# dmMaze/comic-text-detector

Measured on AMD Instinct MI355X. Metric: pages/sec at 1024x1024 bs=32 (end-to-end detector, device-resident pages), higher is better.
Workload: dtype f16

## Files before the change

### comic-text-detector_amd/_lib.py

```python
from __future__ import annotations

import ctypes as C
import os
import subprocess

_HERE = os.path.dirname(os.path.abspath(__file__))
LIB_PATH = os.path.join(_HERE, "libctd_hip.so")
SELFTEST_PATH = os.path.join(_HERE, "ctd_selftest")

ABI_VERSION = 6
OK = 0
PREC_F32, PREC_F16, PREC_F32S = 0, 1, 2
ACT = {"none": 0, "silu": 1, "leaky": 2, "relu": 3, "sigmoid": 4}
IN_NCHW_F32, IN_NHWC_U8 = 0, 1
(OP_INPUT, OP_CONV, OP_CONVT, OP_MAXPOOL, OP_AVGPOOL2, OP_DETECT, OP_EXPORT, OP_STEM, OP_SEG_FINAL,
 OP_DB_UP) = range(1, 11)
OUT_MASK, OUT_LINES = 0, 1


class CtdTensor(C.Structure):
    _fields_ = [("channels", C.c_int32), ("log2_down", C.c_int32), ("dtype", C.c_int32)]


class CtdOp(C.Structure):
    _fields_ = [
# ... 47 lines not shown
    "ctd_nms_workspace_bytes": (C.c_size_t, [_i32, _i32]),
    "ctd_nms": (_i32, [_vp, _i32, _i32, _i32, _f, _f, _i32, _i32, _f, _vp, _vp, _vp, C.c_size_t, _vp]),
    "ctd_db_step": (_i32, [_vp, _i32, _i32, _i32, _f, _vp, _vp, _f, _vp]),
    "ctd_ccl_workspace_bytes": (C.c_size_t, [_i32, _i32, _i32]),
    "ctd_ccl": (_i32, [_vp, _i32, _i32, _i32, _i32, _i32, _vp, _vp, _vp, _i32, _vp, C.c_size_t, _vp]),
    "ctd_ccl_dual": (_i32, [_vp, _i32, _i32, _i32, _i32, _vp, _vp, _vp, _vp, _vp, _vp, _vp, _i32, _vp, C.c_size_t, _vp]),
    "ctd_resize_linear_u8": (_i32, [_vp, _i32, _i32, _i32, _vp, _i32, _i32, _i32, _i32, _vp]),
    "ctd_db_boxes": (_i32, [_vp, _vp, _vp, _i32, _vp, _vp, _i32, _i32, _i32, _i32, C.c_double, _vp, _vp, C.POINTER(_i32)]),
    "ctd_tail_create": (_i32, [C.POINTER(_vp), _i32]),
    "ctd_tail_destroy": (None, [_vp]),
    "ctd_tail_stream": (_vp, [_vp]),
    "ctd_tail_run": (_i32, [_vp, _i32, _i32, _i32, _vp, _i32, _i32, _vp, _vp, _i64, _vp, C.POINTER(CtdTailPage),
                            C.POINTER(CtdTailParams), _vp, _vp, _vp]),
    "ctd_tail_timings": (_i32, [_vp, C.POINTER(C.c_double)]),
    "ctd_tail_refine_paths": (_i32, [_vp, C.POINTER(_i32)]),
    "ctd_tail_db_boxes": (_i32, [_vp, _i32, _i32, _i32, _vp, _i64, _vp, _i32, C.c_double]),
    "ctd_tail_refine": (_i32, [_vp, _i32, C.POINTER(CtdTailPage), _vp, _vp, _vp, _i32, _i32, _vp, _vp]),
    "ctd_tail_page_counts": (_i32, [_vp, _i32, C.POINTER(_i32), C.POINTER(_i32), C.POINTER(_i32), C.POINTER(_i32),
                                    C.POINTER(_i32)]),
    "ctd_tail_page_fetch": (_i32, [_vp, _i32, _vp, _vp, _vp, _vp, _vp, _vp, _vp, _vp]),
    "ctd_tail_batch_counts": (_i32, [_vp, _vp]),
    "ctd_tail_batch_fetch": (_i32, [_vp, _vp, _vp, _vp]),
    "ctd_tail_pack_records": (_i32, [_vp, _i32, _i32, _vp]),
    "ctd_tail_set_threads": (_i32, [_vp, _i32]),
    "ctd_db_boxes_compact": (_i32, [_i32, _i32, _i32, _vp, _vp, _vp, _vp, _vp, _i32, _vp, _vp, _vp, _vp, _vp, _vp, _vp, _vp,
                                    _vp, _i32, C.c_double, _vp, _vp, C.POINTER(_i32)]),
    "ctd_topk_colors": (_i32, [_vp, _vp]),
    "ctd_otsu_from_hist": (_i32, [_vp]),
    "ctd_inrange_bounds": (None, [C.c_double, C.c_double, C.POINTER(_i32), C.POINTER(_i32)]),
    "ctd_group_output": (_i32, [_vp, _vp, _i32, _vp, _i32, _i32, _i32, _vp, _i32, _vp, _i32, _vp, _i32, _vp, _i32,
# ... 70 lines not shown
```

### comic-text-detector_amd/csrc/engine.hip

```cpp
#include <algorithm>
#include <cmath>
#include <cstdio>
#include <cstdlib>
#include <cstring>
#include <string>
#include <vector>

#include "kernels.h"

namespace {

thread_local std::string g_err;

int fail(int code, const std::string& msg) {
  g_err = msg;
  return code;
}

#define HIP_TRY(expr)                                                                              \
  do {                                                                                             \
    hipError_t _e = (expr);                                                                        \
    if (_e != hipSuccess)                                                                          \
      return fail(CTD_ERR_HIP, std::string(#expr) + ": " + hipGetErrorString(_e));                 \
  } while (0)
// ... 1024 lines not shown

int ctd_fail_msg(int code, const std::string& msg) { return fail(code, msg); }
extern int g_tail_priority;
extern int g_tail_cus, g_tail_cu_first;
extern long long g_tail_dma_min;
#ifdef CTD_MEASURE_KNOBS
extern int g_tail_skip_pages;
extern int g_tail_ablate;
#endif
extern int g_tail_chain;
extern int g_tail_fused_rounds;
extern long long g_tail_fused_max_pix;
extern int g_tail_lds, g_tail_lds_rcap, g_tw_lds_runs_x10, g_tw_lds_threads;
extern long long g_tail_lds_cls0, g_tail_lds_cls1;
extern long long g_tail_lds_max_bytes;

extern "C" {

const char* ctd_last_error(void) { return g_err.c_str(); }
int32_t ctd_abi_version(void) { return CTD_ABI_VERSION; }

int ctd_device_info(int32_t device, char* name, int32_t* cu_count, int64_t* hbm_bytes) {
  hipDeviceProp_t p;
  HIP_TRY(hipGetDeviceProperties(&p, device));
  if (name) { std::strncpy(name, p.name, 255); name[255] = 0; }
  if (cu_count) *cu_count = p.multiProcessorCount;
  if (hbm_bytes) *hbm_bytes = (int64_t)p.totalGlobalMem;
  int arch = 0;
  const char* g = std::strstr(p.gcnArchName, "gfx");
  if (g) arch = std::atoi(g + 3);
// ... 137 lines not shown
  }
  return CTD_OK;
}

int64_t ctd_engine_workspace_bytes(const ctd_engine* e) { return e ? (int64_t)e->arena_bytes : 0; }
int32_t ctd_engine_arena_generation(const ctd_engine* e) { return e ? e->arena_gen : -1; }

int ctd_tuning_set(const char* key, int64_t value) {
  const std::string k = key ? key : "";
  if (k == "fuse") g_fuse = (int)value;
  else if (k == "tail_max_blocks") g_tail_max_blocks = (int)std::max<int64_t>(1, value);
  else if (k == "tail_chain") g_tail_chain = (int)value;
  else if (k == "tail_fused_rounds") g_tail_fused_rounds = (int)value;
  else if (k == "tail_fused_max_pix") g_tail_fused_max_pix = value;
  else if (k == "tail_lds") g_tail_lds = (int)value;
  else if (k == "tail_lds_rcap") g_tail_lds_rcap = (int)value;
  else if (k == "tail_lds_max_bytes") g_tail_lds_max_bytes = value;
  else if (k == "tail_lds_runs_x10") g_tw_lds_runs_x10 = (int)std::max<int64_t>(1, value);
  else if (k == "tail_lds_threads") g_tw_lds_threads = (int)value;
  else if (k == "tail_lds_cls0") g_tail_lds_cls0 = value;
  else if (k == "tail_lds_cls1") g_tail_lds_cls1 = value;
  else if (k == "tail_dma_min") g_tail_dma_min = value;
#ifdef CTD_MEASURE_KNOBS
  else if (k == "tail_skip_page_download") g_tail_skip_pages = value != 0;
  else if (k == "tail_ablate") g_tail_ablate = (int)value;
#endif
  else if (k == "tail_priority") g_tail_priority = (int)value;
  else if (k == "tail_cus") g_tail_cus = (int)value;
  else if (k == "tail_cu_first") g_tail_cu_first = (int)value;
  else if (k == "no_reuse") g_no_reuse = (int)value;
// ... 89 lines not shown
```

### comic-text-detector_amd/csrc/tail.h

```cpp
#pragma once
#include "ctd_common.h"

extern int g_tail_max_blocks;

struct DbcTables {
  int B, H, W, cap, rcap;
  const float* prob;
  long long prob_stride;
  const int* lab;
  const int* n_f;
  const int* n_b;
  const int* st_f;
  const int* st_b;
  const int* first_f;
  const int* first_b;
  int* par_f;
  int* par_b;
  int* off_f;
  int* off_b;
  int* hdr;
  int* row_lo;
  int* row_hi;
  double* sum_f;
  double* sum_b;
  double* ring_sum;
  int* ring_cnt;
};
void launch_dbc(const DbcTables& t, hipStream_t st);

struct TWin {
  const uint8_t* img;
  const uint8_t* mask;
  uint8_t* out;
  int img_w, mask_w, out_w;
  int x1, y1, w, h;
  int mx, my;
  int band0, nband;
};
struct TRule {
  int kind;
  int lo, hi;
};
struct TBand {
// ... 49 lines not shown
```

### comic-text-detector_amd/csrc/tail.hip

```cpp
#include <algorithm>
#include <atomic>
#include <chrono>
#include <mutex>
#include <cmath>
#include <cstring>
#include <string>
#include <thread>
#include <vector>

#include "host_refine.h"
#include "kernels.h"
#include "tail.h"

int ctd_fail_msg(int code, const std::string& msg);
int g_tail_priority = 1;
int g_tail_cus = 0, g_tail_cu_first = 0;

#define T_TRY(expr)                                                                                  \
  do {                                                                                               \
    hipError_t e_ = (expr);                                                                          \
    if (e_ != hipSuccess) return ctd_fail_msg(CTD_ERR_HIP, std::string(#expr) + ": " + hipGetErrorString(e_)); \
  } while (0)

namespace {
// ... 56 lines not shown
  std::vector<double> dist;
  std::vector<int16_t> db_boxes;
  std::vector<float> db_scores;
  std::vector<int32_t> yolo;
  std::vector<int32_t> yolo_cls;
  std::vector<float> yolo_conf;
};

struct WinReq {
  int page, x1, y1, x2, y2;
};

constexpr int kMaxDet = 300;
constexpr int kCompCap = 1 << 16;
constexpr int kRowCap = 1 << 18;

inline size_t align_up(size_t v, size_t a) { return (v + a - 1) / a * a; }

template <class F>
void parallel_for(int n, int max_threads, F f) {
  const int nt = std::min(max_threads, n);
  if (nt <= 1) {
    for (int i = 0; i < n; ++i) f(i);
    return;
  }
  std::atomic<int> next{0};
  auto work = [&]() {
    for (int i; (i = next.fetch_add(1)) < n;) f(i);
  };
  std::vector<std::thread> th;
  th.reserve(nt - 1);
  for (int k = 1; k < nt; ++k) th.emplace_back(work);
  work();
  for (auto& x : th) x.join();
}

}
int g_tail_chain = 1;
int g_tail_fused_rounds = 1;
long long g_tail_fused_max_pix = 100000;
int g_tail_lds = 1, g_tail_lds_rcap = 0;
long long g_tail_lds_max_bytes = 150 << 10;
long long g_tail_lds_cls0 = 40 << 10, g_tail_lds_cls1 = 80 << 10;
namespace {
struct ChainState {
  std::mutex mu;
  hipEvent_t last = nullptr;
  hipEvent_t ring[16] = {};
  unsigned next = 0;
};
constexpr int kChainDevices = 64;
inline ChainState* chain_state(int device) {
  static ChainState states[kChainDevices];
  return device >= 0 && device < kChainDevices ? &states[device] : nullptr;
}
struct GpuChain {
  hipStream_t st;
  ChainState* cs;
// ... 77 lines not shown
    return nullptr;
  }
  if (a.type == hipMemoryTypeHost && a.devicePointer) return a.devicePointer;
  return nullptr;
}

inline double now_ms() {
  return std::chrono::duration<double, std::milli>(std::chrono::steady_clock::now().time_since_epoch()).count();
}

}

struct ctd_tail {
  int device = 0;
  hipStream_t st = nullptr;
  DevBuf d_dets, d_nms_ws, d_lab_f, d_ccl_ws, d_ccl_small, d_dbc_i, d_dbc_d, d_rows, d_pmask, d_refined;
  DevBuf d_wins, d_rules, d_bands, d_hist, d_sums, d_canvas, d_clab, d_cstats, d_cnt, d_merged, d_mlab, d_mstats, d_cnt2, d_small, d_crop;
  DevBuf d_wins_c, d_bands_c, d_lds;
  PinBuf h_dets, h_hdr, h_tab, h_pmask, h_refined, h_hist, h_sums, h_wins, h_rules, h_bands, h_small, h_lab;
  PinBuf h_wins_c, h_bands_c, h_lds;
  int B = 0;
  std::vector<ctd_tail_page> pages;
  std::vector<size_t> poff;
  std::vector<uint8_t*> hmask;
  size_t ptotal = 0;
  std::vector<PageOut> out;
  double ms_stage[10] = {0, 0, 0, 0, 0, 0, 0, 0, 0, 0};
  double ms_db_wait = 0;
  double ms_sub[5] = {0, 0, 0, 0, 0};
  int host_threads = 8;
  int n_lds = 0, n_canvas = 0, n_ovf = 0;
  long long lds_per_block = 64 << 10;
  double ms_lds_wait = 0;
};

namespace {

struct Packed {
  std::vector<int> x, y;
  int W = 0, H = 0;
};
void shelf_pack(const std::vector<int>& w, const std::vector<int>& h, int min_width, Packed& out) {
  const int n = (int)w.size();
  out.x.assign(n, 0);
  out.y.assign(n, 0);
  int cw = min_width;
  for (int i = 0; i < n; ++i) cw = std::max(cw, w[i]);
  std::vector<int> order(n);
// ... 390 lines not shown
  const double w0 = now_ms();
  T_TRY(hipStreamSynchronize(st));
  t->ms_sub[3] = now_ms() - w0;
  return CTD_OK;
}

struct DbStage {
  int B = 0, Hn = 0, Wn = 0;
  const float* prob = nullptr;
  long long prob_stride = 0;
  int *lab = nullptr, *n_f = nullptr, *n_b = nullptr, *st_f = nullptr, *st_b = nullptr;
  int *first_f = nullptr, *first_b = nullptr, *par_f = nullptr, *par_b = nullptr, *off_f = nullptr, *off_b = nullptr;
  int *hdr = nullptr, *ring_cnt = nullptr, *row_lo = nullptr, *row_hi = nullptr;
  double *sum_f = nullptr, *sum_b = nullptr, *ring_sum = nullptr;
  int* hhdr = nullptr;
};

int db_enqueue(ctd_tail* t, DbStage& d, int B, int Hn, int Wn, const float* prob_dev, long long prob_stride,
               const uint8_t* bitmap_dev, Batch& pre, Batch& post) {
  hipStream_t st = t->st;
  const size_t hw = (size_t)Hn * Wn;
  const int cap = kCompCap, rcap = kRowCap;
  d.B = B, d.Hn = Hn, d.Wn = Wn, d.prob = prob_dev, d.prob_stride = prob_stride;
  GET(t->d_lab_f, (size_t)B * hw * 4, int, lab);
  GET(t->d_ccl_ws, ccl_workspace_bytes(B, Hn, Wn), uint8_t, ccl_ws);
  const size_t bc = (size_t)B * cap;
  GET(t->d_dbc_i, (2 * (size_t)B + 10 * bc + 6 * bc + 4 * (size_t)B + bc) * 4, int, ti);
  d.lab = lab;
  d.n_f = ti;
  d.n_b = d.n_f + B;
  d.st_f = d.n_b + B;
  d.st_b = d.st_f + 5 * bc;
  d.first_f = d.st_b + 5 * bc;
  d.first_b = d.first_f + bc;
  d.par_f = d.first_b + bc;
  d.par_b = d.par_f + bc;
  d.off_f = d.par_b + bc;
  d.off_b = d.off_f + bc;
  d.hdr = d.off_b + bc;
  d.ring_cnt = d.hdr + 4 * (size_t)B;
  GET(t->d_dbc_d, 3 * bc * 8, double, td);
  d.sum_f = td, d.sum_b = td + bc, d.ring_sum = td + 2 * bc;
  GET(t->d_rows, 2 * (size_t)B * rcap * 4, int, rows);
  d.row_lo = rows, d.row_hi = rows + (size_t)B * rcap;
  pre.fill(td, 0, 3 * bc * 8);
  pre.fill(d.ring_cnt, 0, bc * 4);
  pre.flush();
  launch_ccl_dual(bitmap_dev, B, Hn, Wn, 0, lab, d.n_f, d.n_b, d.st_f, d.st_b, d.first_f, d.first_b, cap, ccl_ws, st);
  DbcTables dt;
  dt.B = B, dt.H = Hn, dt.W = Wn, dt.cap = cap, dt.rcap = rcap;
  dt.prob = prob_dev, dt.prob_stride = prob_stride;
  dt.lab = lab, dt.n_f = d.n_f, dt.n_b = d.n_b, dt.st_f = d.st_f, dt.st_b = d.st_b;
  dt.first_f = d.first_f, dt.first_b = d.first_b, dt.par_f = d.par_f, dt.par_b = d.par_b, dt.off_f = d.off_f;
  dt.off_b = d.off_b, dt.hdr = d.hdr, dt.row_lo = d.row_lo, dt.row_hi = d.row_hi, dt.sum_f = d.sum_f, dt.sum_b = d.sum_b;
  dt.ring_sum = d.ring_sum, dt.ring_cnt = d.ring_cnt;
  launch_dbc(dt, st);
  GET(t->h_hdr, (size_t)B * 4 * 4, int, hhdr);
  d.hhdr = hhdr;
  T_TRY(post.d2h(hhdr, d.hdr, (size_t)B * 16));
  T_TRY(hipGetLastError());
  return CTD_OK;
}

int db_collect(ctd_tail* t, const DbStage& d, const ctd_tail_params* prm) {
  hipStream_t st = t->st;
  const int B = d.B, Hn = d.Hn, Wn = d.Wn, cap = kCompCap, rcap = kRowCap;
  const size_t hw = (size_t)Hn * Wn;
  const int* hhdr = d.hhdr;
  int nfm = 0, nbm = 0, rwm = 0;
  for (int b = 0; b < B; ++b)
    nfm = std::max(nfm, hhdr[4 * b]), nbm = std::max(nbm, hhdr[4 * b + 1]), rwm = std::max(rwm, std::min(hhdr[4 * b + 2], rcap));
// ... 59 lines not shown
    int nbox = 0;
    const int rc = ctd_db_boxes_compact(Wn, Hn, hhdr[4 * b], h_st_f + (size_t)b * nf * 5, h_first_f + (size_t)b * nf,
                                        h_par_f + (size_t)b * nf, h_off_f + (size_t)b * nf, h_sum_f + (size_t)b * nf,
                                        hhdr[4 * b + 1], h_st_b + (size_t)b * nb * 5, h_first_b + (size_t)b * nb,
                                        h_par_b + (size_t)b * nb, h_off_b + (size_t)b * nb, h_sum_b + (size_t)b * nb,
                                        h_ring_sum + (size_t)b * nb, h_ring_cnt + (size_t)b * nb, h_row_lo + (size_t)b * nr,
                                        h_row_hi + (size_t)b * nr, maxc, prm->unclip_ratio, po.db_boxes.data(),
                                        po.db_scores.data(), &nbox);
    if (rc) err = rc;
    po.db_boxes.resize((size_t)nbox * 8);
    po.db_scores.resize(nbox);
  });
  if (err) return ctd_fail_msg(err, "ctd_db_boxes_compact failed");
  std::vector<int16_t> boxes((size_t)std::max(maxc, 1) * 8);
  std::vector<float> scores((size_t)std::max(maxc, 1));
  for (int b = 0; b < B; ++b) {
    if (!hhdr[4 * b + 3]) continue;
    PageOut& po = t->out[b];
    int nbox = 0;
    {
      std::vector<int32_t> lab_host_f(hw), lab_host_b(hw);
      std::vector<float> prob_h(hw);
      int nfb[2];
      T_TRY(hipMemcpyAsync(nfb, d.n_f + b, 4, hipMemcpyDeviceToHost, st));
      T_TRY(hipMemcpyAsync(nfb + 1, d.n_b + b, 4, hipMemcpyDeviceToHost, st));
      T_TRY(hipMemcpyAsync(lab_host_f.data(), d.lab + (size_t)b * hw, hw * 4, hipMemcpyDeviceToHost, st));
      T_TRY(hipMemcpyAsync(prob_h.data(), d.prob + (size_t)b * d.prob_stride, hw * 4, hipMemcpyDeviceToHost, st));
      T_TRY(hipStreamSynchronize(st));
      for (size_t i = 0; i < hw; ++i) {
        const int32_t l = lab_host_f[i];
        lab_host_f[i] = l > 0 ? l : 0;
        lab_host_b[i] = l < 0 ? -l : 0;
      }
      std::vector<int32_t> sf((size_t)nfb[0] * 5), sb((size_t)nfb[1] * 5);
      auto stats_of = [&](const std::vector<int32_t>& lab, std::vector<int32_t>& s, int n) {
        for (int l = 0; l < n; ++l) {
          int32_t* q = s.data() + 5 * (size_t)l;
          q[0] = Wn, q[1] = Hn, q[2] = -1, q[3] = -1, q[4] = 0;
        }
        for (int y = 0; y < Hn; ++y)
          for (int x = 0; x < Wn; ++x) {
// ... 47 lines not shown
  }
  int smem = 0;
  if (hipDeviceGetAttribute(&smem, hipDeviceAttributeMaxSharedMemoryPerBlock, device) == hipSuccess && smem > 0) t->lds_per_block = smem;
  *out = t;
  return CTD_OK;
}

void ctd_tail_destroy(ctd_tail* t) {
  if (!t) return;
  (void)hipSetDevice(t->device);
  if (t->st) {
    (void)hipStreamSynchronize(t->st);
    (void)hipStreamDestroy(t->st);
  }
  DevBuf* dv[] = {&t->d_dets, &t->d_nms_ws, &t->d_lab_f, &t->d_ccl_ws, &t->d_ccl_small, &t->d_dbc_i, &t->d_dbc_d,
                  &t->d_rows, &t->d_pmask, &t->d_refined, &t->d_wins, &t->d_rules, &t->d_bands, &t->d_hist, &t->d_sums,
                  &t->d_canvas, &t->d_clab, &t->d_cstats, &t->d_cnt, &t->d_merged, &t->d_mlab, &t->d_mstats, &t->d_cnt2,
                  &t->d_small, &t->d_crop, &t->d_wins_c, &t->d_bands_c, &t->d_lds};
  for (DevBuf* d : dv) d->release();
  PinBuf* pv[] = {&t->h_dets, &t->h_hdr, &t->h_tab, &t->h_pmask, &t->h_refined, &t->h_hist, &t->h_sums, &t->h_wins,
                  &t->h_rules, &t->h_bands, &t->h_small, &t->h_lab, &t->h_wins_c, &t->h_bands_c, &t->h_lds};
  for (PinBuf* p : pv) p->release();
  delete t;
}

void* ctd_tail_stream(ctd_tail* t) { return t ? (void*)t->st : nullptr; }

static int drained(ctd_tail* t, int rc) {
  if (rc != CTD_OK && t && t->st) (void)hipStreamSynchronize(t->st);
  return rc;
}
// ... 186 lines not shown
int ctd_tail_timings(const ctd_tail* t, double* ms16) {
  if (!t || !ms16) return ctd_fail_msg(CTD_ERR_INVALID, "null argument");
  std::memcpy(ms16, t->ms_stage, sizeof(t->ms_stage));
  ms16[10] = t->ms_db_wait;
  for (int i = 0; i < 5; ++i) ms16[11 + i] = t->ms_sub[i];
  ms16[15] = t->ms_lds_wait;
  return CTD_OK;
}

int ctd_tail_refine_paths(const ctd_tail* t, int32_t* counts3) {
  if (!t || !counts3) return ctd_fail_msg(CTD_ERR_INVALID, "null argument");
  counts3[0] = t->n_lds, counts3[1] = t->n_canvas, counts3[2] = t->n_ovf;
  return CTD_OK;
}

static int tail_db_boxes_impl(ctd_tail* t, int32_t B, int32_t Hn, int32_t Wn, const float* prob_dev, int64_t prob_stride,
                             const uint8_t* bitmap_dev, int32_t max_candidates, double unclip_ratio) {
  if (!t || !prob_dev || !bitmap_dev || B < 1 || Hn < 1 || Wn < 1) return ctd_fail_msg(CTD_ERR_INVALID, "bad arguments");
  T_TRY(hipSetDevice(t->device));
  t->B = B;
  t->out.assign(B, PageOut());
  DbStage db;
  Batch pre(t->st), post(t->st);
  if (int rc = db_enqueue(t, db, B, Hn, Wn, prob_dev, prob_stride, bitmap_dev, pre, post)) return rc;
  post.flush();
  T_TRY(hipGetLastError());
  T_TRY(hipStreamSynchronize(t->st));
  ctd_tail_params prm;
  std::memset(&prm, 0, sizeof(prm));
  prm.max_candidates = max_candidates;
// ... 138 lines not shown
```

### comic-text-detector_amd/tail.py

```python
from __future__ import annotations

import ctypes as C
import threading
from typing import List, Optional, Sequence, Tuple

import numpy as np
import torch

from . import _lib as L
from .textblock import BLK_DTYPE, BlockList, TextBlock, blocks_from_batch, blocks_from_records


def _pinned_u8(h: int, w: int) -> np.ndarray:
    return torch.empty((h, w), dtype=torch.uint8, pin_memory=True).numpy()


def _pinned_pages(shapes) -> List[np.ndarray]:
    sizes = [h * w for h, w in shapes]
    buf = torch.empty((sum(sizes),), dtype=torch.uint8, pin_memory=True).numpy()
    out, off = [], 0
    for (h, w), n in zip(shapes, sizes):
        out.append(buf[off: off + n].reshape(h, w))
        off += n
    return out
# ... 142 lines not shown
        return out

    def timings(self) -> dict:
        ms = (C.c_double * 16)()
        L.check(self._lib.ctd_tail_timings(self._h, ms), "ctd_tail_timings")
        keys = ("enqueue1", "wait1", "db_tables+geometry", "yolo+group_output", "refine_wait_hist", "refine_wait_xor",
                "refine_host+enqueue", "undetected", "final_wait+copies", "total", "db_table_wait", "enq1_nms+buffers",
                "enq1_labelling+tables", "enq1_mask_copies", "final_wait_only", "refine_wait_merge")
        return {k: round(v, 3) for k, v in zip(keys, ms)}

    def refine_paths(self) -> dict:
        c = (C.c_int32 * 3)()
        L.check(self._lib.ctd_tail_refine_paths(self._h, c), "ctd_tail_refine_paths")
        return {"lds": int(c[0]), "canvas": int(c[1]), "overflow": int(c[2])}

    def db_boxes(self, prob: torch.Tensor, bitmap: torch.Tensor, max_candidates=1000, unclip_ratio=1.5):
        B, Hn, Wn = bitmap.shape
        prob = prob.float().contiguous()
        bitmap = bitmap.contiguous()
        torch.cuda.current_stream(self.device).synchronize()
        L.check(self._lib.ctd_tail_db_boxes(self._h, B, Hn, Wn, prob.data_ptr(), prob.stride(0), bitmap.data_ptr(),
                                            int(max_candidates), float(unclip_ratio)), "ctd_tail_db_boxes")
        boxes, scores = [], []
        for b in range(B):
            nx = C.c_int32()
            L.check(self._lib.ctd_tail_page_counts(self._h, b, None, None, None, C.byref(nx), None), "ctd_tail_page_counts")
            bx = np.empty((nx.value, 4, 2), np.int16)
            sc = np.empty((nx.value,), np.float32)
            L.check(self._lib.ctd_tail_page_fetch(self._h, b, None, None, None, bx.ctypes.data, sc.ctypes.data, None, None,
                                                  None), "ctd_tail_page_fetch")
# ... 91 lines not shown
```

### include/ctd_hip.h

```cpp
#ifndef CTD_HIP_H
#define CTD_HIP_H

#include <stddef.h>
#include <stdint.h>

#ifdef __cplusplus
extern "C" {
#endif

#define CTD_ABI_VERSION 6

#define CTD_OK 0
#define CTD_ERR_INVALID (-1)
#define CTD_ERR_HIP (-2)
#define CTD_ERR_UNSUPPORTED (-3)
#define CTD_ERR_NOMEM (-4)

#define CTD_PREC_F32 0
#define CTD_PREC_F16 1
#define CTD_PREC_F32S 2

#define CTD_ACT_NONE 0
#define CTD_ACT_SILU 1
#define CTD_ACT_LEAKY 2
#define CTD_ACT_RELU 3
// ... 110 lines not shown
  int32_t pad_;
} ctd_tail_params;

int ctd_tail_create(ctd_tail** out, int32_t device);
void ctd_tail_destroy(ctd_tail* t);
void* ctd_tail_stream(ctd_tail* t);

int ctd_tail_run(ctd_tail* t, int32_t B, int32_t Hn, int32_t Wn, const float* blks_dev, int32_t rows, int32_t no,
                 const uint8_t* mask_u8_dev, const float* prob_dev, int64_t prob_stride, const uint8_t* bitmap_dev,
                 const ctd_tail_page* pages, const ctd_tail_params* prm, uint8_t* const* mask_out,
                 uint8_t* const* refined_out, void* ready_event);

int ctd_tail_timings(const ctd_tail* t, double* ms);

int ctd_tail_refine_paths(const ctd_tail* t, int32_t* counts3);

int ctd_tail_db_boxes(ctd_tail* t, int32_t B, int32_t Hn, int32_t Wn, const float* prob_dev, int64_t prob_stride,
                      const uint8_t* bitmap_dev, int32_t max_candidates, double unclip_ratio);

int ctd_tail_refine(ctd_tail* t, int32_t n_pages, const ctd_tail_page* pages, const uint8_t* const* masks_host,
                    const int32_t* blk_xyxy, const int32_t* blk_counts, int32_t refine_mode, int32_t keep_undetected_mask,
                    uint8_t* const* mask_out, uint8_t* const* refined_out);

int ctd_tail_page_counts(const ctd_tail* t, int32_t page, int32_t* n_blocks, int32_t* n_lines, int32_t* n_dist,
                         int32_t* n_db_boxes, int32_t* n_yolo);
struct ctd_blk;
int ctd_tail_page_fetch(const ctd_tail* t, int32_t page, struct ctd_blk* blocks, int32_t* lines, double* dist,
                        int16_t* db_boxes, float* db_scores, int32_t* yolo_xyxy, int32_t* yolo_cls, float* yolo_conf);

int ctd_tail_batch_counts(const ctd_tail* t, int32_t* counts);
// ... 57 lines not shown
```

Baseline: 3173.

## Add run-length bit-packed connected-component path for DB box extraction

Replaces the per-pixel dual CCL plus compact-stats pass for DB boxes with a run-based pipeline. It bit-packs the bitmap, finds runs via transition words and a prefix scan, unions runs across rows, and computes component stats, offsets and probability sums per run. This is meant to cut the per-pixel label traffic and the work of the union-find and stats passes. Pages that overflow the run capacity fall back to a per-page plane CCL, at the cost of extra kernels and workspace.

```diff
diff --git a/comic-text-detector_amd/_lib.py b/comic-text-detector_amd/_lib.py
--- a/comic-text-detector_amd/_lib.py
+++ b/comic-text-detector_amd/_lib.py
@@ -8,7 +8,7 @@
 LIB_PATH = os.path.join(_HERE, "libctd_hip.so")
 SELFTEST_PATH = os.path.join(_HERE, "ctd_selftest")
 
-ABI_VERSION = 6
+ABI_VERSION = 7
 OK = 0
 PREC_F32, PREC_F16, PREC_F32S = 0, 1, 2
 ACT = {"none": 0, "silu": 1, "leaky": 2, "relu": 3, "sigmoid": 4}
@@ -86,6 +86,7 @@
                             C.POINTER(CtdTailParams), _vp, _vp, _vp]),
     "ctd_tail_timings": (_i32, [_vp, C.POINTER(C.c_double)]),
     "ctd_tail_refine_paths": (_i32, [_vp, C.POINTER(_i32)]),
+    "ctd_tail_db_paths": (_i32, [_vp, C.POINTER(_i32)]),
     "ctd_tail_db_boxes": (_i32, [_vp, _i32, _i32, _i32, _vp, _i64, _vp, _i32, C.c_double]),
     "ctd_tail_refine": (_i32, [_vp, _i32, C.POINTER(CtdTailPage), _vp, _vp, _vp, _i32, _i32, _vp, _vp]),
     "ctd_tail_page_counts": (_i32, [_vp, _i32, C.POINTER(_i32), C.POINTER(_i32), C.POINTER(_i32), C.POINTER(_i32),
diff --git a/comic-text-detector_amd/csrc/engine.hip b/comic-text-detector_amd/csrc/engine.hip
--- a/comic-text-detector_amd/csrc/engine.hip
+++ b/comic-text-detector_amd/csrc/engine.hip
@@ -1062,6 +1062,7 @@
 extern int g_tail_lds, g_tail_lds_rcap, g_tw_lds_runs_x10, g_tw_lds_threads;
 extern long long g_tail_lds_cls0, g_tail_lds_cls1;
 extern long long g_tail_lds_max_bytes;
+extern int g_tail_db_runs;
 
 extern "C" {
 
@@ -1229,6 +1230,7 @@
   else if (k == "tail_fused_rounds") g_tail_fused_rounds = (int)value;
   else if (k == "tail_fused_max_pix") g_tail_fused_max_pix = value;
   else if (k == "tail_lds") g_tail_lds = (int)value;
+  else if (k == "tail_db_runs") g_tail_db_runs = (int)value;
   else if (k == "tail_lds_rcap") g_tail_lds_rcap = (int)value;
   else if (k == "tail_lds_max_bytes") g_tail_lds_max_bytes = value;
   else if (k == "tail_lds_runs_x10") g_tw_lds_runs_x10 = (int)std::max<int64_t>(1, value);
diff --git a/comic-text-detector_amd/csrc/kernels_dbrun.hip b/comic-text-detector_amd/csrc/kernels_dbrun.hip
--- /dev/null
+++ b/comic-text-detector_amd/csrc/kernels_dbrun.hip
@@ -0,0 +1,439 @@
+#include <hip/amd_detail/amd_hip_unsafe_atomics.h>
+
+#include "tail.h"
+
+namespace {
+
+constexpr int DR_SCAN_T = 1024;
+
+__device__ __forceinline__ int dr_load(const int* parent, int x) {
+  return __hip_atomic_load(parent + x, __ATOMIC_RELAXED, __HIP_MEMORY_SCOPE_AGENT);
+}
+__device__ __forceinline__ int dr_find(const int* parent, int x) {
+  int p = dr_load(parent, x);
+  while (p != x) {
+    x = p;
+    p = dr_load(parent, x);
+  }
+  return x;
+}
+__device__ __forceinline__ void dr_union(int* parent, int a, int b) {
+  while (true) {
+    a = dr_find(parent, a);
+    b = dr_find(parent, b);
+    if (a == b) return;
+    if (a > b) { const int t = a; a = b; b = t; }
+    const int old = atomicMin(parent + b, a);
+    if (old == b) return;
+    b = old;
+  }
+}
+
+__device__ __forceinline__ unsigned upto(int k) { return (2u << k) - 1u; }
+__device__ __forceinline__ unsigned valid_mask(int W, int w) { return W - 32 * w >= 32 ? ~0u : (1u << (W - 32 * w)) - 1u; }
+
+__device__ __forceinline__ int run_of(const unsigned* __restrict__ trans, const int* __restrict__ pre, int WW, int y, int x) {
+  const int i = y * WW + (x >> 5);
+  return pre[i] + __popc(trans[i] & upto(x & 31)) - 1;
+}
+
+__device__ __forceinline__ unsigned nib_of(unsigned v) {
+  const unsigned nz = ((((v & 0x7f7f7f7fu) + 0x7f7f7f7fu) | v) & 0x80808080u) >> 7;
+  return ((nz * 0x00204081u) >> 21) & 15u;
+}
+
+template <class T>
+__device__ __forceinline__ T block_scan_excl(T v, T* sh, T* total) {
+  const int lane = threadIdx.x & 63, w = threadIdx.x >> 6;
+  T incl = v;
+  for (int off = 1; off < 64; off <<= 1) {
+    const T u = __shfl_up(incl, off);
+    if (lane >= off) incl += u;
+  }
+  if (lane == 63) sh[w] = incl;
+  __syncthreads();
+  T base = 0, tot = 0;
+  for (int i = 0; i < DR_SCAN_T / 64; ++i) {
+    if (i < w) base += sh[i];
+    tot += sh[i];
+  }
+  *total = tot;
+  __syncthreads();
+  return base + incl - v;
+}
+
+__global__ __launch_bounds__(256) void dbr_pack_kernel(DbrTables r) {
+  const int b = blockIdx.y, W = r.t.W, WW = r.WW, nw = r.t.H * WW;
+  const uint8_t* img = r.img + (size_t)b * r.t.H * W;
+  unsigned* bits = r.bits + (size_t)b * nw;
+  unsigned* trans = r.trans + (size_t)b * nw;
+  for (int i = blockIdx.x * 256 + threadIdx.x; i < nw; i += gridDim.x * 256) {
+    const int y = i / WW, w = i - y * WW, x0 = 32 * w, n = min(32, W - x0);
+    const uint8_t* src = img + y * W + x0;
+    unsigned v = 0;
+    if (n == 32 && (((size_t)src) & 3) == 0) {
+      const unsigned* s4 = (const unsigned*)src;
+#pragma unroll
+      for (int k = 0; k < 8; ++k) v |= nib_of(s4[k]) << (4 * k);
+    } else {
+      for (int k = 0; k < n; ++k) v |= (src[k] ? 1u : 0u) << k;
+    }
+    const unsigned prev = w > 0 ? (src[-1] ? 1u : 0u) : (~v & 1u);
+    bits[i] = v;
+    trans[i] = (v ^ ((v << 1) | prev)) & valid_mask(W, w);
+  }
+}
+
+__global__ __launch_bounds__(DR_SCAN_T) void dbr_scan_kernel(DbrTables r) {
+  __shared__ int sh[DR_SCAN_T / 64];
+  const int b = blockIdx.x, nw = r.t.H * r.WW;
+  const unsigned* trans = r.trans + (size_t)b * nw;
+  int* pre = r.pre + (size_t)b * nw;
+  const int per = (nw + DR_SCAN_T - 1) / DR_SCAN_T;
+  const int i0 = min((int)threadIdx.x * per, nw), i1 = min(i0 + per, nw);
+  int s = 0;
+  for (int i = i0; i < i1; ++i) s += __popc(trans[i]);
+  int total;
+  int e = block_scan_excl<int>(s, sh, &total);
+  for (int i = i0; i < i1; ++i) {
+    pre[i] = e;
+    e += __popc(trans[i]);
+  }
+  if (threadIdx.x == 0) r.nrun[b] = total;
+}
+
+__global__ __launch_bounds__(256) void dbr_runs_kernel(DbrTables r) {
+  const int b = blockIdx.y, W = r.t.W, WW = r.WW, nw = r.t.H * WW;
+  if (r.nrun[b] > r.rcap) return;
+  const unsigned* trans = r.trans + (size_t)b * nw;
+  const int* pre = r.pre + (size_t)b * nw;
+  int* p0 = r.p0 + (size_t)b * r.rcap;
+  int* parent = r.parent + (size_t)b * r.rcap;
+  for (int i = blockIdx.x * 256 + threadIdx.x; i < nw; i += gridDim.x * 256) {
+    unsigned tw = trans[i];
+    if (!tw) continue;
+    const int y = i / WW, w = i - y * WW;
+    int id = pre[i];
+    for (; tw; tw &= tw - 1, ++id) {
+      p0[id] = y * W + 32 * w + (__ffs(tw) - 1);
+      parent[id] = id;
+    }
+  }
+}
+
+__device__ __forceinline__ int run_end(const int* __restrict__ p0, int id, int nrun, int y, int W) {
+  if (id + 1 < nrun) {
+    const int q = p0[id + 1];
+    if (q < (y + 1) * W) return q - y * W - 1;
+  }
+  return W - 1;
+}
+
+__global__ __launch_bounds__(256) void dbr_link_kernel(DbrTables r) {
+  const int b = blockIdx.y, W = r.t.W, WW = r.WW, nw = r.t.H * WW;
+  const int nrun = r.nrun[b];
+  if (nrun > r.rcap) return;
+  const unsigned* bits = r.bits + (size_t)b * nw;
+  const unsigned* trans = r.trans + (size_t)b * nw;
+  const int* pre = r.pre + (size_t)b * nw;
+  const int* p0 = r.p0 + (size_t)b * r.rcap;
+  int* parent = r.parent + (size_t)b * r.rcap;
+  for (int id = blockIdx.x * 256 + threadIdx.x; id < nrun; id += gridDim.x * 256) {
+    const int p = p0[id], y = p / W, x0 = p - y * W;
+    if (y == 0) continue;
+    const int x1 = run_end(p0, id, nrun, y, W);
+    const unsigned fg = (bits[y * WW + (x0 >> 5)] >> (x0 & 31)) & 1u;
+    const int a = max(x0 - (int)fg, 0), e = min(x1 + (int)fg, W - 1);
+    const int up = (y - 1) * WW;
+    for (int w = a >> 5; w <= (e >> 5); ++w) {
+      const unsigned bw = bits[up + w], tw = trans[up + w];
+      unsigned m = (fg ? bw : ~bw) & valid_mask(W, w);
+      if (w == (a >> 5)) m &= ~0u << (a & 31);
+      if (w == (e >> 5)) m &= upto(e & 31);
+      const int pw = pre[up + w];
+      while (m) {
+        const int k = __ffs(m) - 1;
+        dr_union(parent, id, pw + __popc(tw & upto(k)) - 1);
+        const unsigned nt = tw & ~upto(k);
+        if (!nt) break;
+        m &= ~0u << (__ffs(nt) - 1);
+      }
+    }
+  }
+}
+
+__global__ __launch_bounds__(256) void dbr_flatten_kernel(DbrTables r) {
+  const int b = blockIdx.y;
+  const int nrun = r.nrun[b];
+  if (nrun > r.rcap) return;
+  int* parent = r.parent + (size_t)b * r.rcap;
+  for (int id = blockIdx.x * 256 + threadIdx.x; id < nrun; id += gridDim.x * 256) {
+    const int root = dr_find(parent, id);
+    if (root != id) __hip_atomic_store(parent + id, root, __ATOMIC_RELAXED, __HIP_MEMORY_SCOPE_AGENT);
+  }
+}
+
+__global__ __launch_bounds__(DR_SCAN_T) void dbr_rank_kernel(DbrTables r) {
+  __shared__ unsigned long long sh[DR_SCAN_T / 64];
+  const int b = blockIdx.x, W = r.t.W, WW = r.WW, cap = r.t.cap;
+  const int nrun = r.nrun[b];
+  int* n_f = const_cast<int*>(r.t.n_f);
+  int* n_b = const_cast<int*>(r.t.n_b);
+  if (nrun > r.rcap) {
+    if (threadIdx.x == 0) n_f[b] = 0, n_b[b] = 0;
+    return;
+  }
+  const unsigned* bits = r.bits + (size_t)b * r.t.H * WW;
+  const int* p0 = r.p0 + (size_t)b * r.rcap;
+  const int* parent = r.parent + (size_t)b * r.rcap;
+  int* cid = r.cid + (size_t)b * r.rcap;
+  int* first_f = const_cast<int*>(r.t.first_f) + (size_t)b * cap;
+  int* first_b = const_cast<int*>(r.t.first_b) + (size_t)b * cap;
+  int* st_f = const_cast<int*>(r.t.st_f) + (size_t)b * cap * 5;
+  int* st_b = const_cast<int*>(r.t.st_b) + (size_t)b * cap * 5;
+  const int per = (nrun + DR_SCAN_T - 1) / DR_SCAN_T;
+  const int i0 = min((int)threadIdx.x * per, nrun), i1 = min(i0 + per, nrun);
+  unsigned long long s = 0;
+  for (int id = i0; id < i1; ++id) {
+    if (parent[id] != id) continue;
+    const int p = p0[id], y = p / W, x = p - y * W;
+    s += ((bits[y * WW + (x >> 5)] >> (x & 31)) & 1u) ? 1ull : (1ull << 32);
+  }
+  unsigned long long total;
+  unsigned long long e = block_scan_excl<unsigned long long>(s, sh, &total);
+  for (int id = i0; id < i1; ++id) {
+    if (parent[id] != id) continue;
+    const int p = p0[id], y = p / W, x = p - y * W;
+    const bool fg = (bits[y * WW + (x >> 5)] >> (x & 31)) & 1u;
+    const int k = fg ? (int)(e & 0xffffffffull) : (int)(e >> 32);
+    e += fg ? 1ull : (1ull << 32);
+    cid[id] = k + 1;
+    if (k < cap) {
+      (fg ? first_f : first_b)[k] = p;
+      int* q = (fg ? st_f : st_b) + 5 * k;
+      q[0] = W, q[1] = r.t.H, q[2] = -1, q[3] = -1, q[4] = 0;
+    }
+  }
+  if (threadIdx.x == 0) n_f[b] = (int)(total & 0xffffffffull), n_b[b] = (int)(total >> 32);
+}
+
+__global__ __launch_bounds__(256) void dbr_stats_kernel(DbrTables r) {
+  const int b = blockIdx.y, W = r.t.W, WW = r.WW, cap = r.t.cap;
+  const int nrun = r.nrun[b];
+  if (nrun > r.rcap) return;
+  const unsigned* bits = r.bits + (size_t)b * r.t.H * WW;
+  const int* p0 = r.p0 + (size_t)b * r.rcap;
+  const int* parent = r.parent + (size_t)b * r.rcap;
+  const int* cid = r.cid + (size_t)b * r.rcap;
+  int* st_f = const_cast<int*>(r.t.st_f) + (size_t)b * cap * 5;
+  int* st_b = const_cast<int*>(r.t.st_b) + (size_t)b * cap * 5;
+  for (int id = blockIdx.x * 256 + threadIdx.x; id < nrun; id += gridDim.x * 256) {
+    const int c = cid[parent[id]] - 1;
+    if (c >= cap) continue;
+    const int p = p0[id], y = p / W, x0 = p - y * W;
+    const int x1 = run_end(p0, id, nrun, y, W);
+    const bool fg = (bits[y * WW + (x0 >> 5)] >> (x0 & 31)) & 1u;
+    int* q = (fg ? st_f : st_b) + 5 * c;
+    atomicMin(q + 0, x0);
+    atomicMin(q + 1, y);
+    atomicMax(q + 2, x1);
+    atomicMax(q + 3, y);
+    atomicAdd(q + 4, x1 - x0 + 1);
+  }
+}
+
+__global__ __launch_bounds__(256) void dbr_prep_kernel(DbrTables r) {
+  const int b = blockIdx.y, l = blockIdx.x * 256 + threadIdx.x;
+  const DbcTables& t = r.t;
+  if (r.nrun[b] > r.rcap) return;
+  const int nw = t.H * r.WW;
+  const int nf = min(t.n_f[b], t.cap), nb = min(t.n_b[b], t.cap);
+  const unsigned* trans = r.trans + (size_t)b * nw;
+  const int* pre = r.pre + (size_t)b * nw;
+  const int* parent = r.parent + (size_t)b * r.rcap;
+  const int* cid = r.cid + (size_t)b * r.rcap;
+  const size_t row = (size_t)b * t.cap + l;
+  if (l < nf) {
+    int* s = const_cast<int*>(t.st_f) + row * 5;
+    s[2] -= s[0] - 1, s[3] -= s[1] - 1;
+    const int p = t.first_f[row], y = p / t.W, x = p - y * t.W;
+    t.par_f[row] = x > 0 ? cid[parent[run_of(trans, pre, r.WW, y, x) - 1]] : 0;
+    t.off_f[row] = s[3];
+  }
+  if (l < nb) {
+    int* s = const_cast<int*>(t.st_b) + row * 5;
+    s[2] -= s[0] - 1, s[3] -= s[1] - 1;
+    const bool hole = s[0] > 0 && s[1] > 0 && s[0] + s[2] < t.W && s[1] + s[3] < t.H;
+    const int p = t.first_b[row], y = p / t.W, x = p - y * t.W;
+    t.par_b[row] = hole ? cid[parent[run_of(trans, pre, r.WW, y, x) - 1]] : 0;
+    t.off_b[row] = hole ? s[3] + 2 : 0;
+  }
+}
+
+__global__ __launch_bounds__(DR_SCAN_T) void dbr_offsets_kernel(DbrTables r) {
+  __shared__ int sh[DR_SCAN_T / 64];
+  const DbcTables& t = r.t;
+  const int b = blockIdx.x;
+  const bool run_ovf = r.nrun[b] > r.rcap;
+  const int nf = run_ovf ? 0 : min(t.n_f[b], t.cap), nb = run_ovf ? 0 : min(t.n_b[b], t.cap);
+  int carry = 0;
+  for (int pass = 0; pass < 2; ++pass) {
+    int* a = (pass ? t.off_b : t.off_f) + (size_t)b * t.cap;
+    const int n = pass ? nb : nf;
+    for (int base = 0; base < n; base += DR_SCAN_T) {
+      const int i = base + threadIdx.x;
+      const int v = i < n ? a[i] : 0;
+      int total;
+      const int e = block_scan_excl<int>(v, sh, &total);
+      if (i < n) a[i] = carry + e;
+      carry += total;
+    }
+  }
+  if (threadIdx.x == 0) {
+    int* h = t.hdr + b * 4;
+    h[0] = nf, h[1] = nb, h[2] = carry;
+    h[3] = (run_ovf || t.n_f[b] > t.cap || t.n_b[b] > t.cap || carry > t.rcap) ? 1 : 0;
+  }
+}
+
+__global__ __launch_bounds__(256) void dbr_init_kernel(DbrTables r) {
+  const DbcTables& t = r.t;
+  const int b = blockIdx.y;
+  const int* h = t.hdr + b * 4;
+  if (h[3]) return;
+  const int rows = h[2], nrun = r.nrun[b];
+  const unsigned* bits = r.bits + (size_t)b * t.H * r.WW;
+  const int* p0 = r.p0 + (size_t)b * r.rcap;
+  const int* parent = r.parent + (size_t)b * r.rcap;
+  const int* cid = r.cid + (size_t)b * r.rcap;
+  int* rc = r.rc + (size_t)b * r.rcap;
+  const int n = max(rows, nrun);
+  for (int i = blockIdx.x * 256 + threadIdx.x; i < n; i += gridDim.x * 256) {
+    if (i < rows) t.row_lo[(size_t)b * t.rcap + i] = 0x7fffffff, t.row_hi[(size_t)b * t.rcap + i] = -1;
+    if (i < nrun) {
+      const int c = cid[parent[i]];
+      const int p = p0[i], y = p / t.W, x = p - y * t.W;
+      const bool fg = (bits[y * r.WW + (x >> 5)] >> (x & 31)) & 1u;
+      rc[i] = fg ? c : (t.par_b[(size_t)b * t.cap + c - 1] > 0 ? -c : 0);
+    }
+  }
+}
+
+__global__ __launch_bounds__(256) void dbr_accum_kernel(DbrTables r) {
+  const DbcTables& t = r.t;
+  const int b = blockIdx.y, W = t.W, H = t.H, WW = r.WW, nw = H * WW;
+  if (t.hdr[b * 4 + 3]) return;
+  const unsigned* bits = r.bits + (size_t)b * nw;
+  const unsigned* trans = r.trans + (size_t)b * nw;
+  const int* pre = r.pre + (size_t)b * nw;
+  const int* rc = r.rc + (size_t)b * r.rcap;
+  const float* prob = t.prob + (long long)b * t.prob_stride;
+  const size_t cb = (size_t)b * t.cap, rb = (size_t)b * t.rcap;
+  for (int i = blockIdx.x * 256 + threadIdx.x; i < nw; i += gridDim.x * 256) {
+    const int y = i / WW, w = i - y * WW, x0 = 32 * w, n = min(32, W - x0);
+    const unsigned vm = valid_mask(W, w);
+    const unsigned bw = bits[i], tw = trans[i];
+    const int pw = pre[i];
+    const float* pr = prob + y * W + x0;
+    int id = pw + (int)(tw & 1u) - 1;
+    unsigned rest = tw & ~1u;
+    for (int s = 0; s < n; ++id) {
+      const int e = rest ? __ffs(rest) - 1 : n;
+      rest &= rest - 1;
+      const int v = rc[id];
+      if (v) {
+        double sum = 0.0;
+        for (int k = s; k < e; ++k) sum += (double)pr[k];
+        if (v > 0) {
+          const size_t c = cb + v - 1;
+          unsafeAtomicAdd(t.sum_f + c, sum);
+          const int row = t.off_f[c] + (y - t.st_f[c * 5 + 1]);
+          atomicMin(t.row_lo + rb + row, x0 + s);
+          atomicMax(t.row_hi + rb + row, x0 + e - 1);
+        } else {
+          unsafeAtomicAdd(t.sum_b + cb + (-v) - 1, sum);
+        }
+      }
+      s = e;
+    }
+    const unsigned bg = ~bw & vm;
+    const unsigned lf_in = w > 0 ? (~bits[i - 1] >> 31) : 0u;
+    const unsigned rt_in = w + 1 < WW ? (~bits[i + 1] & valid_mask(W, w + 1) & 1u) << 31 : 0u;
+    const unsigned bg_up = y > 0 ? ~bits[i - WW] & vm : 0u;
+    const unsigned bg_dn = y + 1 < H ? ~bits[i + WW] & vm : 0u;
+    unsigned cand = bw & ((bg << 1) | lf_in | (bg >> 1) | rt_in | bg_up | bg_dn);
+    for (; cand; cand &= cand - 1) {
+      const int k = __ffs(cand) - 1, x = x0 + k;
+      const int lf = rc[pw + __popc(tw & upto(k)) - 1];
+      const int nx[4] = {x - 1, x + 1, x, x}, ny[4] = {y, y, y - 1, y + 1};
+      const bool ok[4] = {x > 0, x + 1 < W, y > 0, y + 1 < H};
+      int hbs[4], prs[4];
+#pragma unroll
+      for (int j = 0; j < 4; ++j) hbs[j] = ok[j] ? -rc[run_of(trans, pre, WW, ny[j], nx[j])] : 0;
+#pragma unroll
+      for (int j = 0; j < 4; ++j) prs[j] = hbs[j] > 0 ? t.par_b[cb + hbs[j] - 1] : -1;
+      int seen[4];
+      int ns = 0;
+      double pv = 0.0;
+#pragma unroll
+      for (int j = 0; j < 4; ++j) {
+        const int hb = hbs[j];
+        if (hb <= 0 || prs[j] != lf) continue;
+        bool dup = false;
+#pragma unroll
+        for (int q = 0; q < 4; ++q) dup |= q < ns && seen[q] == hb;
+        if (dup) continue;
+        if (ns == 0) pv = (double)pr[k];
+        seen[ns++] = hb;
+        unsafeAtomicAdd(t.ring_sum + cb + hb - 1, pv);
+        atomicAdd(t.ring_cnt + cb + hb - 1, 1);
+        const int row = t.off_b[cb + hb - 1] + (y - (t.st_b[(cb + hb - 1) * 5 + 1] - 1));
+        atomicMin(t.row_lo + rb + row, x);
+        atomicMax(t.row_hi + rb + row, x);
+      }
+    }
+  }
+}
+
+inline int page_grid(long long items, int B) {
+  const long long want = (items + 255) / 256;
+  return (int)std::max<long long>(1, std::min<long long>(want, g_tail_max_blocks / std::max(1, B)));
+}
+
+}
+
+size_t dbrun_workspace_bytes(int B, int H, int W, int rcap) {
+  const size_t nw = (size_t)H * ((W + 31) / 32);
+  return ((size_t)B * (3 * nw + 4 * (size_t)rcap) + (size_t)B) * 4;
+}
+
+void launch_dbrun(const DbcTables& t, const uint8_t* img, int rcap, void* ws, hipStream_t st) {
+  DbrTables r;
+  r.t = t;
+  r.img = img;
+  r.WW = (t.W + 31) / 32;
+  r.rcap = rcap;
+  const size_t nw = (size_t)t.H * r.WW, B = (size_t)t.B;
+  int* p = (int*)ws;
+  r.bits = (unsigned*)p, p += B * nw;
+  r.trans = (unsigned*)p, p += B * nw;
+  r.pre = p, p += B * nw;
+  r.p0 = p, p += B * rcap;
+  r.parent = p, p += B * rcap;
+  r.cid = p, p += B * rcap;
+  r.rc = p, p += B * rcap;
+  r.nrun = p;
+  const dim3 gw(page_grid((long long)nw, t.B), t.B);
+  const dim3 gr(page_grid(std::min<long long>((long long)rcap, (long long)nw), t.B), t.B);
+  hipLaunchKernelGGL(dbr_pack_kernel, gw, dim3(256), 0, st, r);
+  hipLaunchKernelGGL(dbr_scan_kernel, dim3(t.B), dim3(DR_SCAN_T), 0, st, r);
+  hipLaunchKernelGGL(dbr_runs_kernel, gw, dim3(256), 0, st, r);
+  hipLaunchKernelGGL(dbr_link_kernel, gr, dim3(256), 0, st, r);
+  hipLaunchKernelGGL(dbr_flatten_kernel, gr, dim3(256), 0, st, r);
+  hipLaunchKernelGGL(dbr_rank_kernel, dim3(t.B), dim3(DR_SCAN_T), 0, st, r);
+  hipLaunchKernelGGL(dbr_stats_kernel, gr, dim3(256), 0, st, r);
+  hipLaunchKernelGGL(dbr_prep_kernel, dim3((t.cap + 255) / 256, t.B), dim3(256), 0, st, r);
+  hipLaunchKernelGGL(dbr_offsets_kernel, dim3(t.B), dim3(DR_SCAN_T), 0, st, r);
+  hipLaunchKernelGGL(dbr_init_kernel, gr, dim3(256), 0, st, r);
+  hipLaunchKernelGGL(dbr_accum_kernel, gw, dim3(256), 0, st, r);
+}
diff --git a/comic-text-detector_amd/csrc/tail.h b/comic-text-detector_amd/csrc/tail.h
--- a/comic-text-detector_amd/csrc/tail.h
+++ b/comic-text-detector_amd/csrc/tail.h
@@ -27,6 +27,22 @@
   int* ring_cnt;
 };
 void launch_dbc(const DbcTables& t, hipStream_t st);
+
+struct DbrTables {
+  DbcTables t;
+  const uint8_t* img;
+  int WW, rcap;
+  unsigned* bits;
+  unsigned* trans;
+  int* pre;
+  int* p0;
+  int* parent;
+  int* cid;
+  int* rc;
+  int* nrun;
+};
+size_t dbrun_workspace_bytes(int B, int H, int W, int rcap);
+void launch_dbrun(const DbcTables& t, const uint8_t* img, int rcap, void* ws, hipStream_t st);
 
 struct TWin {
   const uint8_t* img;
diff --git a/comic-text-detector_amd/csrc/tail.hip b/comic-text-detector_amd/csrc/tail.hip
--- a/comic-text-detector_amd/csrc/tail.hip
+++ b/comic-text-detector_amd/csrc/tail.hip
@@ -94,6 +94,7 @@
 constexpr int kMaxDet = 300;
 constexpr int kCompCap = 1 << 16;
 constexpr int kRowCap = 1 << 18;
+constexpr int kRunCap = 1 << 18;
 
 inline size_t align_up(size_t v, size_t a) { return (v + a - 1) / a * a; }
 
@@ -122,6 +123,7 @@
 int g_tail_lds = 1, g_tail_lds_rcap = 0;
 long long g_tail_lds_max_bytes = 150 << 10;
 long long g_tail_lds_cls0 = 40 << 10, g_tail_lds_cls1 = 80 << 10;
+int g_tail_db_runs = 1;
 namespace {
 struct ChainState {
   std::mutex mu;
@@ -229,7 +231,7 @@
 struct ctd_tail {
   int device = 0;
   hipStream_t st = nullptr;
-  DevBuf d_dets, d_nms_ws, d_lab_f, d_ccl_ws, d_ccl_small, d_dbc_i, d_dbc_d, d_rows, d_pmask, d_refined;
+  DevBuf d_dets, d_nms_ws, d_lab_f, d_ccl_ws, d_ccl_small, d_dbc_i, d_dbc_d, d_rows, d_pmask, d_refined, d_dbr;
   DevBuf d_wins, d_rules, d_bands, d_hist, d_sums, d_canvas, d_clab, d_cstats, d_cnt, d_merged, d_mlab, d_mstats, d_cnt2, d_small, d_crop;
   DevBuf d_wins_c, d_bands_c, d_lds;
   PinBuf h_dets, h_hdr, h_tab, h_pmask, h_refined, h_hist, h_sums, h_wins, h_rules, h_bands, h_small, h_lab;
@@ -247,6 +249,7 @@
   int n_lds = 0, n_canvas = 0, n_ovf = 0;
   long long lds_per_block = 64 << 10;
   double ms_lds_wait = 0;
+  int n_db_runs = 0, n_db_planes = 0;
 };
 
 namespace {
@@ -667,6 +670,8 @@
   int *hdr = nullptr, *ring_cnt = nullptr, *row_lo = nullptr, *row_hi = nullptr;
   double *sum_f = nullptr, *sum_b = nullptr, *ring_sum = nullptr;
   int* hhdr = nullptr;
+  const uint8_t* bitmap = nullptr;
+  bool runs = false;
 };
 
 int db_enqueue(ctd_tail* t, DbStage& d, int B, int Hn, int Wn, const float* prob_dev, long long prob_stride,
@@ -675,8 +680,16 @@
   const size_t hw = (size_t)Hn * Wn;
   const int cap = kCompCap, rcap = kRowCap;
   d.B = B, d.Hn = Hn, d.Wn = Wn, d.prob = prob_dev, d.prob_stride = prob_stride;
-  GET(t->d_lab_f, (size_t)B * hw * 4, int, lab);
-  GET(t->d_ccl_ws, ccl_workspace_bytes(B, Hn, Wn), uint8_t, ccl_ws);
+  d.bitmap = bitmap_dev, d.runs = g_tail_db_runs != 0;
+  const int run_cap = (int)std::min<size_t>(kRunCap, hw);
+  int* lab = nullptr;
+  uint8_t *ccl_ws = nullptr, *dbr_ws = nullptr;
+  if (d.runs) {
+    if (int rc_ = t->d_dbr.get(dbrun_workspace_bytes(B, Hn, Wn, run_cap), (void**)&dbr_ws)) return rc_;
+  } else {
+    if (int rc_ = t->d_lab_f.get((size_t)B * hw * 4, (void**)&lab)) return rc_;
+    if (int rc_ = t->d_ccl_ws.get(ccl_workspace_bytes(B, Hn, Wn), (void**)&ccl_ws)) return rc_;
+  }
   const size_t bc = (size_t)B * cap;
   GET(t->d_dbc_i, (2 * (size_t)B + 10 * bc + 6 * bc + 4 * (size_t)B + bc) * 4, int, ti);
   d.lab = lab;
@@ -699,7 +712,7 @@
   pre.fill(td, 0, 3 * bc * 8);
   pre.fill(d.ring_cnt, 0, bc * 4);
   pre.flush();
-  launch_ccl_dual(bitmap_dev, B, Hn, Wn, 0, lab, d.n_f, d.n_b, d.st_f, d.st_b, d.first_f, d.first_b, cap, ccl_ws, st);
+  if (!d.runs) launch_ccl_dual(bitmap_dev, B, Hn, Wn, 0, lab, d.n_f, d.n_b, d.st_f, d.st_b, d.first_f, d.first_b, cap, ccl_ws, st);
   DbcTables dt;
   dt.B = B, dt.H = Hn, dt.W = Wn, dt.cap = cap, dt.rcap = rcap;
   dt.prob = prob_dev, dt.prob_stride = prob_stride;
@@ -707,7 +720,8 @@
   dt.first_f = d.first_f, dt.first_b = d.first_b, dt.par_f = d.par_f, dt.par_b = d.par_b, dt.off_f = d.off_f;
   dt.off_b = d.off_b, dt.hdr = d.hdr, dt.row_lo = d.row_lo, dt.row_hi = d.row_hi, dt.sum_f = d.sum_f, dt.sum_b = d.sum_b;
   dt.ring_sum = d.ring_sum, dt.ring_cnt = d.ring_cnt;
-  launch_dbc(dt, st);
+  if (d.runs) launch_dbrun(dt, bitmap_dev, run_cap, dbr_ws, st);
+  else launch_dbc(dt, st);
   GET(t->h_hdr, (size_t)B * 4 * 4, int, hhdr);
   d.hhdr = hhdr;
   T_TRY(post.d2h(hhdr, d.hdr, (size_t)B * 16));
@@ -797,17 +811,34 @@
   if (err) return ctd_fail_msg(err, "ctd_db_boxes_compact failed");
   std::vector<int16_t> boxes((size_t)std::max(maxc, 1) * 8);
   std::vector<float> scores((size_t)std::max(maxc, 1));
+  t->n_db_runs = t->n_db_planes = 0;
   for (int b = 0; b < B; ++b) {
-    if (!hhdr[4 * b + 3]) continue;
+    if (!hhdr[4 * b + 3]) {
+      ++(d.runs ? t->n_db_runs : t->n_db_planes);
+      continue;
+    }
+    ++t->n_db_planes;
     PageOut& po = t->out[b];
     int nbox = 0;
     {
+      const int* lab_dev = d.runs ? nullptr : d.lab + (size_t)b * hw;
+      if (d.runs) {
+        int* lab1;
+        uint8_t* ws1;
+        if (int rc_ = t->d_lab_f.get(hw * 4, (void**)&lab1)) return rc_;
+        if (int rc_ = t->d_ccl_ws.get(ccl_workspace_bytes(1, Hn, Wn), (void**)&ws1)) return rc_;
+        const size_t o = (size_t)b * cap;
+        launch_ccl_dual(d.bitmap + (size_t)b * hw, 1, Hn, Wn, 0, lab1, d.n_f + b, d.n_b + b, d.st_f + 5 * o, d.st_b + 5 * o,
+                        d.first_f + o, d.first_b + o, cap, ws1, st);
+        T_TRY(hipGetLastError());
+        lab_dev = lab1;
+      }
       std::vector<int32_t> lab_host_f(hw), lab_host_b(hw);
       std::vector<float> prob_h(hw);
       int nfb[2];
       T_TRY(hipMemcpyAsync(nfb, d.n_f + b, 4, hipMemcpyDeviceToHost, st));
       T_TRY(hipMemcpyAsync(nfb + 1, d.n_b + b, 4, hipMemcpyDeviceToHost, st));
-      T_TRY(hipMemcpyAsync(lab_host_f.data(), d.lab + (size_t)b * hw, hw * 4, hipMemcpyDeviceToHost, st));
+      T_TRY(hipMemcpyAsync(lab_host_f.data(), lab_dev, hw * 4, hipMemcpyDeviceToHost, st));
       T_TRY(hipMemcpyAsync(prob_h.data(), d.prob + (size_t)b * d.prob_stride, hw * 4, hipMemcpyDeviceToHost, st));
       T_TRY(hipStreamSynchronize(st));
       for (size_t i = 0; i < hw; ++i) {
@@ -885,7 +916,7 @@
     (void)hipStreamDestroy(t->st);
   }
   DevBuf* dv[] = {&t->d_dets, &t->d_nms_ws, &t->d_lab_f, &t->d_ccl_ws, &t->d_ccl_small, &t->d_dbc_i, &t->d_dbc_d,
-                  &t->d_rows, &t->d_pmask, &t->d_refined, &t->d_wins, &t->d_rules, &t->d_bands, &t->d_hist, &t->d_sums,
+                  &t->d_dbr, &t->d_rows, &t->d_pmask, &t->d_refined, &t->d_wins, &t->d_rules, &t->d_bands, &t->d_hist, &t->d_sums,
                   &t->d_canvas, &t->d_clab, &t->d_cstats, &t->d_cnt, &t->d_merged, &t->d_mlab, &t->d_mstats, &t->d_cnt2,
                   &t->d_small, &t->d_crop, &t->d_wins_c, &t->d_bands_c, &t->d_lds};
   for (DevBuf* d : dv) d->release();
@@ -1102,6 +1133,12 @@
   return CTD_OK;
 }
 
+int ctd_tail_db_paths(const ctd_tail* t, int32_t* counts2) {
+  if (!t || !counts2) return ctd_fail_msg(CTD_ERR_INVALID, "null argument");
+  counts2[0] = t->n_db_runs, counts2[1] = t->n_db_planes;
+  return CTD_OK;
+}
+
 static int tail_db_boxes_impl(ctd_tail* t, int32_t B, int32_t Hn, int32_t Wn, const float* prob_dev, int64_t prob_stride,
                              const uint8_t* bitmap_dev, int32_t max_candidates, double unclip_ratio) {
   if (!t || !prob_dev || !bitmap_dev || B < 1 || Hn < 1 || Wn < 1) return ctd_fail_msg(CTD_ERR_INVALID, "bad arguments");
diff --git a/comic-text-detector_amd/tail.py b/comic-text-detector_amd/tail.py
--- a/comic-text-detector_amd/tail.py
+++ b/comic-text-detector_amd/tail.py
@@ -180,6 +180,11 @@
         L.check(self._lib.ctd_tail_refine_paths(self._h, c), "ctd_tail_refine_paths")
         return {"lds": int(c[0]), "canvas": int(c[1]), "overflow": int(c[2])}
 
+    def db_paths(self) -> dict:
+        c = (C.c_int32 * 2)()
+        L.check(self._lib.ctd_tail_db_paths(self._h, c), "ctd_tail_db_paths")
+        return {"runs": int(c[0]), "planes": int(c[1])}
+
     def db_boxes(self, prob: torch.Tensor, bitmap: torch.Tensor, max_candidates=1000, unclip_ratio=1.5):
         B, Hn, Wn = bitmap.shape
         prob = prob.float().contiguous()
diff --git a/include/ctd_hip.h b/include/ctd_hip.h
--- a/include/ctd_hip.h
+++ b/include/ctd_hip.h
@@ -8,7 +8,7 @@
 extern "C" {
 #endif
 
-#define CTD_ABI_VERSION 6
+#define CTD_ABI_VERSION 7
 
 #define CTD_OK 0
 #define CTD_ERR_INVALID (-1)
@@ -149,6 +149,8 @@
 int ctd_tail_timings(const ctd_tail* t, double* ms);
 
 int ctd_tail_refine_paths(const ctd_tail* t, int32_t* counts3);
+
+int ctd_tail_db_paths(const ctd_tail* t, int32_t* counts2);
 
 int ctd_tail_db_boxes(ctd_tail* t, int32_t B, int32_t Hn, int32_t Wn, const float* prob_dev, int64_t prob_stride,
                       const uint8_t* bitmap_dev, int32_t max_candidates, double unclip_ratio);
```

New measurement: 956.8. -69.8%, worse.
